# omrijsharon/FpyV

Measured on AMD Instinct MI355X. Metric: env-steps/sec at N=1.05M drones, dt=1ms; 1/2/4/8 GPU + CPU ref, higher is better.
Workload: dtype f32

## Files before the change

__graft_entry__.py:

```python
import os
import subprocess
import sys

REPO = os.path.dirname(os.path.abspath(__file__))
if REPO not in sys.path:
    sys.path.insert(0, REPO)

HIP_SRC = os.path.join(REPO, "fpyv_amd", "csrc", "fpv_hip.hip")
HIP_SRCS = [HIP_SRC, os.path.join(REPO, "fpyv_amd", "csrc", "fpv_phys.hip"), os.path.join(REPO, "fpyv_amd", "csrc", "fpv_gate.hip"),
            os.path.join(REPO, "fpyv_amd", "csrc", "fpv_range.hip")]
HIP_SRCS_ALL = HIP_SRCS + [os.path.join(REPO, "fpyv_amd", "csrc", "fpv_depth.hip")]
HIP_SRCS_BUILD = HIP_SRCS_ALL + [os.path.join(REPO, "fpyv_amd", "csrc", "fpv_chase.hip")]
HIP_SRCS_LINK = HIP_SRCS_BUILD + [os.path.join(REPO, "fpyv_amd", "csrc", "fpv_pursuit.hip")]
HIP_SRCS_PNS = HIP_SRCS_LINK + [os.path.join(REPO, "fpyv_amd", "csrc", "fpv_pns.hip")]
HIP_LIB = os.path.join(REPO, "fpyv_amd", "libfpv_hip.so")
HIPCC_FLAGS = ["-O3", "--offload-arch=gfx950", "-ffp-contract=off", "-fno-slp-vectorize", "-std=c++17", "-shared",
               "-fPIC", "-Wall", "-Wextra", "-mllvm", "-amdgpu-kernarg-preload-count=6"]


def _stale(target, sources):
    if not os.path.isfile(target):
        return True
    t = os.path.getmtime(target)
    return any(os.path.getmtime(s) > t for s in sources)


def build(force: bool = False) -> None:
    csrc = os.path.join(REPO, "fpyv_amd", "csrc")
    deps = [os.path.join(csrc, f) for f in os.listdir(csrc)] + [os.path.join(REPO, "include", "fpv_abi.h")]
    if force or _stale(HIP_LIB, deps):
        hipcc = os.environ.get("HIPCC", "/opt/rocm/bin/hipcc")
        subprocess.run([hipcc] + HIPCC_FLAGS + ["-o", HIP_LIB] + HIP_SRCS_PNS, check=True)
    subprocess.run(["make", "-C", os.path.join(REPO, "oracle")] + (["-B"] if force else []), check=True,
                   stdout=subprocess.DEVNULL)
    import fpyv_amd
    from fpyv_amd import _lib
    L = _lib.lib()
    missing = [s for s in _lib.EXPORTS if not hasattr(L, s)]
    assert not missing, f"libfpv_hip.so lacks {missing}"
    assert fpyv_amd.__version__


def smoke() -> None:
    import numpy as np
    import torch
    from fpyv_amd import load_params, sticks
    from fpyv_amd.env import DroneBatch
    from oracle import lane_model, oracle
    sys.path.insert(0, os.path.join(REPO, "tests"))
    from parity import assert_parity, soa_vs_oracle

    assert torch.cuda.is_available(), "smoke() needs a GPU"
    p = load_params(fps=1000)
    n, steps = 256, 200
    acts = sticks.ema_noise(steps, range(n), seed=7)
    a = torch.from_numpy(acts).to("cuda:0")
    env, fused = DroneBatch(p, n, device="cuda:0"), DroneBatch(p, n, device="cuda:0")
    env.reset(); fused.reset()
    for t in range(steps):
        env.step(a[t], return_imu=False)
    fused.rollout(a)
    torch.cuda.synchronize()
    got = env.state.cpu().numpy()
    assert torch.equal(env.state, fused.state), "k-step kernel != k single steps"

# ... 14 lines not shown
```

fpyv_amd/_lib.py:

```python
from __future__ import annotations

import ctypes as C
import os
from typing import Optional


_HERE = os.path.dirname(os.path.abspath(__file__))
LIB_PATH = os.path.join(_HERE, "libfpv_hip.so")

FPV_ABI_VERSION = 9
FPV_OK = 0
FPV_MODE_DRONE, FPV_MODE_RACER = 0, 1
FPV_DRONE_ROWS, FPV_RACER_ROWS = 14, 29
FPV_FLAG_AUTO_RESET = 1
FPV_FLAG_GROUND = 2
FPV_FLAG_FP16_STATE = 4
FPV_FLAG_STICK_NOISE = 8
FPV_FLAG_RESET_JITTER = 16
RESET_POSE_ROWS = 10
FPV_PHYS_ROWS = 13
FPV_PHYS_INPUTS = 10
PHYS_IN_MASS, PHYS_IN_C3, PHYS_IN_CD_X, PHYS_IN_RATES_LAG, PHYS_IN_THRUST_LAG = 0, 1, 5, 8, 9
FPV_MAX_GATES = 64
FPV_GATE_FLOATS = 16
GATE_SHAPES = {"rectangle": 0, "circle": 1, "half_circle": 2}
GATE_EVENT_NONE, GATE_EVENT_PASS, GATE_EVENT_MISS, GATE_EVENT_FINISH = 0, 1, 2, 3
GATE_OBS_ROWS = 6
FPV_MAX_RAYS = 32
FPV_DEPTH_MAX_SIDE = 128
DEPTH_ENCODINGS = {"metres": 0, "u8": 1}
FPV_CHASE_MAX_SIDE = 16384
CHASE_FRAMES = {"world": 0, "drone": 1}
CHASE_MODES = {"level": 0, "frontarget": 1}
FPV_TGT_ROWS = 8
TGT_CX, TGT_CY, TGT_CZ, TGT_PATH_R, TGT_RADIUS, TGT_PREV_DIST, TGT_COUNT, TGT_SPAWNS = range(8)
FPV_TGT_FRESH = 0x80000000
FPV_PURSUIT_OBS = 7
FPV_PURSUIT_MAX_RESOLUTION = 65536
FPV_HALF_PAIR_ROWS = 5
FPV_HALF_HALVES = 11
FPV_OBS_AOS_DIM = 16

PX, PY, PZ, VX, VY, VZ, QW, QX, QY, QZ, RX, RY, RZ, THRUST = range(14)
R_OMEGA, R_IERR, R_LERR, R_FIRST, R_OMEGA_LO, R_IERR_LO, R_DFILT = 10, 13, 16, 19, 20, 23, 26

EXPORTS = ("fpv_abi_version", "fpv_sizeof", "fpv_state_rows", "fpv_algorithmic_bytes", "fpv_handle_algorithmic_bytes", "fpv_create", "fpv_destroy",
           "fpv_reset", "fpv_step", "fpv_rollout", "fpv_step_n", "fpv_rollout_graph", "fpv_return_triple", "fpv_widen_state", "fpv_set_params", "fpv_set_step_counter", "fpv_get_step_counter", "fpv_set_rotation", "fpv_get_rotation", "fpv_recommended_ld",
           "fpv_recommended_ld_device", "fpv_check_cache_model", "fpv_device_cache_model", "fpv_get_cache_model",
           "fpv_diag_stream_copy", "fpv_diag_stream_copy_wide", "fpv_diag_busy", "fpv_diag_xcd_map", "fpv_pid_reset", "fpv_pid_call", "fpv_comm_unique_id", "fpv_comm_create", "fpv_comm_destroy", "fpv_comm_info",
           "fpv_allgather_done", "fpv_allgather_f32", "fpv_last_error",
           "fpv_error_name", "fpv_encoding_id", "fpv_reset_pose_sample",
           "fpv_physics_rows", "fpv_physics_derive", "fpv_physics_sample", "fpv_set_physics", "fpv_get_physics",
           "fpv_gates_derive", "fpv_set_gates", "fpv_gate_eval",
           "fpv_rays_derive", "fpv_range_scan", "fpv_range_eval",
           "fpv_camera_derive", "fpv_depth_render", "fpv_depth_eval",
           "fpv_chase_derive", "fpv_chase_guide", "fpv_chase_eval",
           "fpv_pursuit_derive", "fpv_pursuit_sample", "fpv_pursuit_step", "fpv_pursuit_reset", "fpv_pursuit_eval",
           "fpv_pns_derive", "fpv_pns_guide", "fpv_pns_eval")


class FpvParams(C.Structure):
    _fields_ = [
        ("struct_size", C.c_uint32), ("mode", C.c_uint32), ("flags", C.c_uint32), ("racer_omega_dt", C.c_uint32),
        ("dt", C.c_double), ("gravity", C.c_double), ("mass", C.c_double), ("max_rates", C.c_double),
        ("rates_transition_rate", C.c_double), ("thrust_transition_rate", C.c_double),
        ("thrust_poly", C.c_double * 4),
        ("drag_coefficients", C.c_double * 3), ("cross_section_areas", C.c_double * 3),
        ("air_density", C.c_double),
        ("motor_xy", (C.c_double * 2) * 4),
        ("init_position", C.c_double * 3), ("init_velocity", C.c_double * 3), ("init_quat", C.c_double * 4),
        ("ceiling", C.c_double), ("goal", C.c_double * 3),
        ("racer_mass", C.c_double), ("racer_inertia", C.c_double * 3), ("racer_pid", (C.c_double * 3) * 3),
        ("racer_velocity_damping", C.c_double),
        ("motor_radius", C.c_double), ("ground_spring", C.c_double), ("ground_damping", C.c_double),
        ("noise_transition", C.c_double), ("noise_gain", C.c_double),
        ("noise_seed", C.c_uint64), ("drone_id_offset", C.c_uint64),
        ("racer_pid_variant", C.c_uint32), ("_reserved0", C.c_uint32),
        ("pid_integral_clip", C.c_double), ("pid_min_output", C.c_double), ("pid_max_output", C.c_double),
        ("pid_derivative_transition_rate", C.c_double),
        ("reset_pos_range", (C.c_double * 3) * 2), ("reset_vel_range", (C.c_double * 3) * 2),
# ... 211 lines not shown

class FpvError(RuntimeError):
    def __init__(self, code: int, name: str, msg: str):
        super().__init__(f"{name} ({code}): {msg}")
        self.code, self.name = code, name


_lib: Optional[C.CDLL] = None


def lib() -> C.CDLL:
    global _lib
    if _lib is not None:
        return _lib
    if not os.path.isfile(LIB_PATH):
        raise ImportError(f"{LIB_PATH} is missing - build it with `python -c 'import __graft_entry__ as g; g.build()'` "
                          "(hipcc --offload-arch=gfx950).  fpyv_amd has no CPU fallback.")
    import torch
    L = C.CDLL(LIB_PATH, mode=C.RTLD_LOCAL)
    vp, i64, pp, pb = C.c_void_p, C.c_int64, C.POINTER(FpvParams), C.POINTER(FpvBuffers)
    L.fpv_abi_version.restype = C.c_int
    L.fpv_state_rows.argtypes = [C.c_int]
    L.fpv_algorithmic_bytes.argtypes = [C.c_int]
    L.fpv_handle_algorithmic_bytes.argtypes = [vp]
    L.fpv_create.argtypes = [pp, i64, C.c_int, C.POINTER(vp)]
    L.fpv_destroy.argtypes = [vp]
    L.fpv_destroy.restype = None
    L.fpv_reset.argtypes = [vp, pb, vp, vp, vp, vp, vp]
    L.fpv_step.argtypes = [vp, pb, vp]
    L.fpv_rollout.argtypes = [vp, pb, C.c_int, i64, i64, vp]
    L.fpv_rollout_graph.argtypes = [vp, pb, C.c_int, i64, i64, vp]
    L.fpv_step_n.argtypes = [vp, pb, C.c_int, i64, i64, vp]
    L.fpv_return_triple.argtypes = [vp, pb, vp, vp, vp, vp]
    L.fpv_widen_state.argtypes = [vp, pb, vp, i64, vp]
    L.fpv_set_params.argtypes = [vp, pp]
    L.fpv_set_step_counter.argtypes = [vp, C.c_uint64]
    L.fpv_get_step_counter.argtypes = [vp, C.POINTER(C.c_uint64)]
    L.fpv_set_rotation.argtypes = [vp, C.c_int64]
    L.fpv_get_rotation.argtypes = [vp, C.POINTER(C.c_int64)]
    L.fpv_recommended_ld.argtypes = [i64]
    L.fpv_recommended_ld.restype = i64
    L.fpv_recommended_ld_device.argtypes = [i64, C.c_int]
    L.fpv_recommended_ld_device.restype = i64
    L.fpv_check_cache_model.argtypes = [C.c_char_p, C.c_int, i64, C.POINTER(FpvCacheModel)]
    L.fpv_device_cache_model.argtypes = [C.c_int, C.POINTER(FpvCacheModel)]
    L.fpv_get_cache_model.argtypes = [vp, C.POINTER(FpvCacheModel)]
    L.fpv_diag_stream_copy.argtypes = [vp, vp, i64, vp]
    L.fpv_diag_stream_copy_wide.argtypes = [vp, vp, i64, vp]
    L.fpv_diag_busy.argtypes = [C.c_double, vp]
    L.fpv_diag_xcd_map.argtypes = [vp, i64, vp]
    L.fpv_comm_unique_id.argtypes = [vp]
    L.fpv_comm_create.argtypes = [vp, C.c_int, C.c_int, C.c_int, C.POINTER(vp)]
    L.fpv_comm_destroy.argtypes = [vp]
    L.fpv_comm_destroy.restype = None
    L.fpv_comm_info.argtypes = [vp, C.POINTER(C.c_int), C.POINTER(C.c_int), C.POINTER(C.c_int)]
    L.fpv_allgather_done.argtypes = [vp, vp, vp, i64, vp]
    L.fpv_allgather_f32.argtypes = [vp, vp, vp, i64, vp]
    L.fpv_pid_reset.argtypes = [vp, i64, i64, vp, C.c_int, vp]
    L.fpv_pid_call.argtypes = [C.POINTER(FpvPidParams), vp, i64, i64, vp, vp, C.c_float, vp, vp, C.c_int, vp]
    L.fpv_last_error.restype = C.c_char_p
    L.fpv_error_name.argtypes = [C.c_int]
    L.fpv_error_name.restype = C.c_char_p
    L.fpv_encoding_id.argtypes = [C.c_int]
    L.fpv_encoding_id.restype = C.c_char_p
    L.fpv_sizeof.argtypes = [C.c_int]
    L.fpv_reset_pose_sample.argtypes = [pp, C.c_uint64, C.c_uint64, C.c_int, vp, vp]
# ... 51 lines not shown
```

fpyv_amd/csrc/fpv_hip.hip:

```cpp
#include <hip/hip_runtime.h>

#include <dlfcn.h>
#include <math.h>
#include <stdint.h>
#include <stdio.h>
#include <stdlib.h>
#include <string.h>

#include <algorithm>
#include <mutex>
#include <new>
#include <string>
#include <vector>
#include <type_traits>

#include "../../include/fpv_abi.h"
#include "fpv_addr.h"
#include "fpv_exp.h"
#include "fpv_derive.h"
#include "fpv_math.h"
#include "fpv_kernels.h"
#include "fpv_range.h"
#include "fpv_depth.h"
#include "fpv_chase.h"
// ... 668 lines not shown
    fpv_params_t P;
    int64_t n;
    int device;
    int mode;
    FpvResetJitter rj;
    uint64_t launches;
    int64_t rot_blocks = 0, start_block = 0, rot_request = -1;
    fpv_cache_model_t cache;
    hipGraph_t graph = nullptr;
    hipGraphExec_t graph_exec = nullptr;
    std::vector<hipGraphNode_t> graph_nodes;
    std::string graph_shape_key, graph_ptr_key;
    const float* phys = nullptr;
    int64_t phys_ld = 0;
    int phys_rows_last = 0;
    bool gates = false;
    FpvGateArgs ga = {};
};

extern "C" __attribute__((weak, visibility("hidden"))) void* fpv_phys_step_kernel(int noise, int obj);
extern "C" __attribute__((weak, visibility("hidden"))) void* fpv_phys_roll_kernel(int noise, int obj);
extern "C" __attribute__((weak, visibility("hidden"))) void* fpv_gate_step_kernel(void);
extern "C" __attribute__((weak, visibility("hidden"))) void* fpv_gate_roll_kernel(int noise, int obj);
extern "C" __attribute__((weak, visibility("hidden"))) void* fpv_gate_reset_kernel_fn(void);
extern "C" __attribute__((weak, visibility("hidden"))) void* fpv_range_scan_kernel_fn(void);
extern "C" __attribute__((weak, visibility("hidden"))) void* fpv_depth_render_kernel_fn(int u8);
extern "C" __attribute__((weak, visibility("hidden"))) void* fpv_chase_kernel_fn(int pixel);
extern "C" __attribute__((weak, visibility("hidden"))) void fpv_chase_eval_host(const FpvChaseArgs* A, const float* p, const float* v, const float* q);
extern "C" __attribute__((weak, visibility("hidden"))) void* fpv_pns_kernel_fn(int pixel);
extern "C" __attribute__((weak, visibility("hidden"))) void fpv_pns_eval_host(const FpvPnsArgs* A, const float* p, const float* v, const float* q);
extern "C" __attribute__((weak, visibility("hidden"))) void* fpv_pursuit_kernel_fn(int guide, int reset);
extern "C" __attribute__((weak, visibility("hidden"))) void fpv_pursuit_eval_host(const FpvPursuitArgs* A, const float* p, const float* v, const float* q,
                                                                                  int guide, int reset);

namespace {

enum Family { kPlain, kFp16, kAos, kRacer, kTable, kGate };

int check_combination(const fpv_env* h, Family f, const fpv_buffers_t* b)
{
    struct Rule { bool hit; const char* with; };
    const bool table = f == kTable;
    const auto refuse = [&](std::initializer_list<Rule> rules) -> int {
        for (const Rule& r : rules)
            if (r.hit) return fail(FPV_EINVAL, std::string(table ? "a physics table" : "a gate course") + " cannot be combined with " + r.with);
        return FPV_OK;
    };
    if (!b)
        return refuse({{h->mode != FPV_MODE_DRONE, "Racer mode"}, {(h->K.flags & FPV_FLAG_FP16_STATE) != 0, "fp16 state (FPV_FLAG_FP16_STATE)"},
                       table ? Rule{h->gates, "a gate course (fpv_set_gates)"} : Rule{h->phys != nullptr, "a physics table (fpv_set_physics)"}});
    return refuse({{b->pos_comp != nullptr, "Kahan rows (pos_comp)"}, {b->rotation_override != nullptr, "the guidance override (rotation_override)"},
                   {b->obs_aos != nullptr, "the AoS head (obs_aos)"},
                   {!table && (h->K.flags & FPV_FLAG_STICK_NOISE) && b->objects && b->objects->count > 0, "stick noise AND an object list (either one alone is served)"}});
}

int check_object_count(const fpv_objects_t* in, bool most)
{
    if (in && (in->count < 0 || in->count > FPV_MAX_OBJECTS))
        return fail(FPV_EINVAL, "objects.count out of range" + (most ? " (at most " + std::to_string(FPV_MAX_OBJECTS) + " objects)" : std::string()));
    return FPV_OK;
}

int check_object_types(const fpv_objects_t* in)
{
    for (int k = 0; in && k < in->count; ++k)
        if (in->obj[k].type < FPV_OBJ_GROUND || in->obj[k].type > FPV_OBJ_SPHERE) return fail(FPV_EINVAL, "unknown object type");
// ... 155 lines not shown
};

typedef void (*StepKernel)(float*, const int64_t, const float4*, const int64_t, uint16_t*, const int64_t, const FpvK, const FpvBufD);
typedef void (*RollKernel)(const FpvRollArgs);
typedef void (*GateResetKernel)(uint32_t*, const uint8_t*, const uint8_t*, const uint32_t, const int64_t);
inline int64_t step_grid(int64_t n) { return (n + 8 * kStepBlock - 1) / (8 * kStepBlock) * 8; }

const StepKernel kDroneStep[2][2][2] = {
    {{fpv_drone_step_kernel<false, false, false>, fpv_drone_step_kernel<false, false, true>},
     {fpv_drone_step_kernel<false, true, false>, fpv_drone_step_kernel<false, true, true>}},
    {{fpv_drone_step_kernel<true, false, false>, fpv_drone_step_kernel<true, false, true>},
     {fpv_drone_step_kernel<true, true, false>, fpv_drone_step_kernel<true, true, true>}}};
const StepKernel kDroneStepOverride[2] = {fpv_drone_step_kernel<false, false, false, true>, fpv_drone_step_kernel<false, true, false, true>};
const RollKernel kDroneRoll[2][2][2] = {
    {{fpv_drone_rollout_kernel<false, false, false>, fpv_drone_rollout_kernel<false, false, true>},
     {fpv_drone_rollout_kernel<false, true, false>, fpv_drone_rollout_kernel<false, true, true>}},
    {{fpv_drone_rollout_kernel<true, false, false>, fpv_drone_rollout_kernel<true, false, true>},
     {fpv_drone_rollout_kernel<true, true, false>, fpv_drone_rollout_kernel<true, true, true>}}};
const RollKernel kDroneRollSq[2][2] = {
    {fpv_drone_rollout_kernel<false, false, false, true>, fpv_drone_rollout_kernel<false, false, true, true>},
    {fpv_drone_rollout_kernel<true, false, false, true>, fpv_drone_rollout_kernel<true, false, true, true>}};
const StepKernel kRacerStep[2][2] = {{fpv_racer_step_kernel<false, false>, fpv_racer_step_kernel<false, true>},
                                     {fpv_racer_step_kernel<true, false>, fpv_racer_step_kernel<true, true>}};
const RollKernel kRacerRoll[2][2] = {{fpv_racer_rollout_kernel<false, false>, fpv_racer_rollout_kernel<false, true>},
                                     {fpv_racer_rollout_kernel<true, false>, fpv_racer_rollout_kernel<true, true>}};

enum GraphRoute { kReplay, kToStepN, kToRollout };
struct Plan {
    Family family;
    void* step;
    void* roll;
    bool ground = false;
    GraphRoute graph = kReplay;
};

template <class... P> void* entry(void (*kernel)(P...)) { return reinterpret_cast<void*>(kernel); }

Plan plan_launch(const fpv_env* h, const FpvBufD& d)
{
    const bool noise = (h->K.flags & FPV_FLAG_STICK_NOISE) != 0, fp16 = (h->K.flags & FPV_FLAG_FP16_STATE) != 0;
    const bool obj = d.objs.count > 0, kahan = d.pos_comp != nullptr, aos = d.obs_aos != nullptr, ground = (h->K.flags & FPV_FLAG_GROUND) != 0;
    const bool wide = h->K.r_wide != 0, pidv = h->K.r_pid_variant != 0;
    const bool reset = h->mode == FPV_MODE_DRONE && (d.reset_pose != nullptr || (h->K.flags & FPV_FLAG_RESET_JITTER) != 0);
    const bool sq = !obj && h->K.motor_square && !ground && !reset;
    Plan p;
    if (h->gates) p = {kGate, noise || obj ? nullptr : fpv_gate_step_kernel(), fpv_gate_roll_kernel(noise, obj)};
    else if (h->phys) p = {kTable, fpv_phys_step_kernel(noise, obj), fpv_phys_roll_kernel(noise, obj), ground || obj};
    else if (h->mode != FPV_MODE_DRONE) p = {kRacer, entry(kRacerStep[wide][pidv]), entry(kRacerRoll[wide][pidv])};
    else if (fp16) p = {kFp16, entry(fpv_drone_step_h_kernel), entry(fpv_drone_rollout_h_kernel)};
    else p = {aos ? kAos : kPlain, entry(aos ? fpv_drone_step_aos_kernel : d.rot_over ? kDroneStepOverride[obj] : kDroneStep[noise][obj][kahan]),
              entry(sq ? kDroneRollSq[noise][kahan] : kDroneRoll[noise][obj][kahan])};
    if (reset && !aos) p.step = nullptr;
    p.graph = noise || fp16 || !p.step ? kToStepN : reset ? kToRollout : kReplay;
    return p;
}

void launched(fpv_env* h, const Plan& p, int k)
{
    h->launches += (uint64_t)k;
    if (p.family == kTable) h->phys_rows_last = p.ground ? FPV_PHYS_ROWS : FPV_PHYS_ROWS - 2;
}

int launch_roll(fpv_env* h, const Plan& p, const FpvBufD& d, const FpvRoll& R, hipStream_t s, const char* what)
{
    FpvRollArgs a = {h->K, d, h->n, R};
    a.B.step = h->launches;
    FpvRollPhysArgs pa;
    FpvRollGateArgs ga;
    void* arg = &a;
    if (p.family == kTable) { pa = {a, h->phys, p.ground ? 1 : 0, 0}; arg = &pa; }
    if (p.family == kGate) { ga = {a, h->ga}; arg = &ga; }
    const int rc = launch_args(what, p.roll, blocks_for(h->n, kStepBlock), dim3(kStepBlock), s, &arg);
    if (rc == FPV_OK) launched(h, p, R.k);
    return rc;
}

struct StepLaunch {
    FpvBufD d;
    FpvK K;
    int64_t n_start;
    void* slot5;
    FpvGateArgs ga;
    void* args[9];
    hipKernelNodeParams np;
    StepLaunch(const fpv_env* h, const Plan& p, const FpvBufD& dt, int64_t start)
        : d(dt), K(h->K), n_start(h->n | (start << 32) | (p.ground ? kPhysGroundBit : 0)),
          slot5(p.family == kGate ? (void*)h->ga.word : p.family == kTable ? (void*)const_cast<float*>(h->phys) : (void*)dt.state_h),
          ga(h->ga), args{&d.state, &d.ld, &d.action, &d.action_ld, &slot5, &n_start, &K, &d, &ga}
    {
        memset(&np, 0, sizeof(np));
        np.func = p.step; np.kernelParams = args;
        np.gridDim = dim3((unsigned)step_grid(h->n)); np.blockDim = dim3(kStepBlock);
    }
    StepLaunch(const StepLaunch&) = delete;
    StepLaunch& operator=(const StepLaunch&) = delete;
};

int64_t rotation_blocks(const fpv_env* h, const FpvBufD* d);

int launch_step(fpv_env* h, const Plan& p, const FpvBufD& d, hipStream_t s)
{
    if (!p.step) return launch_roll(h, p, d, FpvRoll{1, 0, 0, 0, 0}, s, "step kernel launch");
    const int64_t nblk = step_grid(h->n);
    h->rot_blocks = rotation_blocks(h, &d);
    const int64_t start = h->rot_blocks > 0 ? h->start_block % nblk : 0;
    StepLaunch L(h, p, d, start);
    L.d.step = h->launches;
    const int rc = launch_args("step kernel launch", L.np.func, L.np.gridDim, L.np.blockDim, s, L.np.kernelParams);
    if (rc != FPV_OK) return rc;
    launched(h, p, 1);
    if (h->rot_blocks > 0) h->start_block = (start + nblk - h->rot_blocks % nblk) % nblk;
    return FPV_OK;
}

template <class... T> std::string bytes_of(const T&... v)
{
    std::string s;
    (s.append(reinterpret_cast<const char*>(&v), sizeof(v)), ...);
    return s;
}

constexpr int kModelXcds = 8, kModelComputeUnits = 256;
constexpr int64_t kModelL2BytesPerXcd = (int64_t)4 << 20;
constexpr int64_t kInfinityCacheBytes = (int64_t)256 << 20;
constexpr int64_t kL2Bytes = (int64_t)kModelXcds * kModelL2BytesPerXcd;

void check_cache_model(const char* arch, int compute_units, int64_t l2_bytes, fpv_cache_model_t* m)
{
    memset(m, 0, sizeof(*m));
    m->struct_size = (uint32_t)sizeof(*m);
    m->compute_units = compute_units;
    m->l2_bytes_per_xcd = l2_bytes;
    snprintf(m->arch, sizeof(m->arch), "%s", arch ? arch : "");
    std::string why;
    if (strncmp(m->arch, "gfx950", 6) != 0 || (m->arch[6] != '\0' && m->arch[6] != ':'))
        why = std::string("architecture '") + m->arch + "' is not gfx950";
    else if (compute_units != kModelComputeUnits)
        why = "the process sees " + std::to_string(compute_units) + " compute units, not " + std::to_string(kModelComputeUnits)
              + " (a compute partition of the chip? the model is eight XCDs of 32 CUs in single-partition mode)";
// ... 983 lines not shown
            const double o = l2_set_overflow(4 * c, blocks);
            if (o < kL2OverflowOk) return c;
            if (o < best) { best = o; best_ld = c; }
        }
    return best_ld;
}

int fpv_reset(fpv_handle_t h, const fpv_buffers_t* b, const uint8_t* mask, const float* position,
              const float* velocity, const float* ypr_deg, void* stream)
{
    int rc = check_buffers(h, b, false);
    if (rc != FPV_OK) return rc;
    const DeviceGuard dev(h->device);
    if (dev.rc != FPV_OK) return dev.rc;
    FpvBufD d = to_device_view(h, b);
    d.step = h->launches;
    rc = launch("reset kernel launch", fpv_reset_kernel, blocks_for(h->n, kBlock), dim3(kBlock), (hipStream_t)stream, h->K, d,
                h->mode, mask, position, velocity, ypr_deg, h->n);
    if (rc != FPV_OK || !h->gates) return rc;
    return launch("gate word reset launch", reinterpret_cast<GateResetKernel>(fpv_gate_reset_kernel_fn()), blocks_for(h->n, kBlock), dim3(kBlock),
                  (hipStream_t)stream, h->ga.word, mask, h->ga.start, h->ga.K.count, h->n);
}

int fpv_step(fpv_handle_t h, const fpv_buffers_t* b, void* stream)
{
    int rc = check_buffers(h, b, true);
    if (rc != FPV_OK) return rc;
    const DeviceGuard dev(h->device);
    if (dev.rc != FPV_OK) return dev.rc;
    const FpvBufD d = to_device_view(h, b);
    return launch_step(h, plan_launch(h, d), d, (hipStream_t)stream);
}

namespace {

void drop_graph(fpv_env* h)
{
    if (h->graph_exec) { (void)hipGraphExecDestroy(h->graph_exec); h->graph_exec = nullptr; }
    if (h->graph) { (void)hipGraphDestroy(h->graph); h->graph = nullptr; }
    h->graph_nodes.clear();
    h->graph_shape_key.clear();
    h->graph_ptr_key.clear();
}

FpvBufD graph_step_view(const fpv_buffers_t* b, const FpvBufD& d0, int t, int64_t action_stride, int64_t out_stride)
{
    FpvBufD d = d0;
    if (b->action) d.action = reinterpret_cast<const float4*>(b->action + (int64_t)t * action_stride);
    if (out_stride) {
        if (b->reward) d.reward = b->reward + (int64_t)t * out_stride;
        if (b->done) d.done = b->done + (int64_t)t * out_stride;
    }
    if (b->done_bits) d.done_bits = reinterpret_cast<unsigned long long*>(b->done_bits) + (int64_t)t * b->done_bits_stride;
    return d;
}

}

int fpv_rollout(fpv_handle_t h, const fpv_buffers_t* b, int k, int64_t action_stride, int64_t out_stride,
                void* stream)
{
    int rc = check_buffers(h, b, true);
    if (rc != FPV_OK) return rc;
    if (k < 0) return fail(FPV_EINVAL, "k must be >= 0");
    if (action_stride % 4) return fail(FPV_EALIGN, "action_stride must keep 16-byte alignment");
    if (b->rotation_override) return fail(FPV_EINVAL, "the guidance override is a per-step input: use fpv_step");
// ... 329 lines not shown
```

fpyv_amd/csrc/fpv_kernels.h:

```cpp
#pragma once

#include <hip/hip_runtime.h>

#include <stdint.h>

#include <type_traits>

#include "../../include/fpv_abi.h"
#include "fpv_addr.h"
#include "fpv_exp.h"
#include "fpv_math.h"
#include "fpv_gate.h"

namespace {

constexpr int kBlock = 256;
constexpr int kStepBlock = FPV_EXP_BLOCK;
static_assert(kStepBlock % 64 == 0 && kStepBlock >= 64 && kStepBlock <= 1024, "whole wave64s");

struct FpvBufD {
    float* state;
    int64_t ld;
    const float4* action;
    float* reward;
// ... 224 lines not shown
    return p;
}

__device__ __forceinline__ void apply_reset_source_k(uint32_t i, uint64_t t, FpvDroneState& s)
{
    float pose[10] = {s.px, s.py, s.pz, s.vx, s.vy, s.vz, s.q.w, s.q.x, s.q.y, s.q.z};
    FpvArgsPtr A = fpv_args_after(s.px);
    const float* tab = A->B.reset_pose;
    if (tab) {
        const int64_t ld = A->B.ld;
#pragma unroll
        for (int r = 0; r < 10; ++r) pose[r] = row_at(ROW(tab, r, ld), i);
    }
    if (A->K.flags & FPV_FLAG_RESET_JITTER) {
#pragma unroll
        for (uint32_t b = 0; b < 3; ++b) {
            const FpvArgsPtr V = fpv_args_after(pose[3 * b]);
            const float lo[3] = {V->B.rj.lo[3 * b], V->B.rj.lo[3 * b + 1], V->B.rj.lo[3 * b + 2]};
            const float span[3] = {V->B.rj.span[3 * b], V->B.rj.span[3 * b + 1], V->B.rj.span[3 * b + 2]};
            fpv_reset_jitter_block(lo, span, V->B.rj.seed_lo, V->B.rj.seed_hi, (((uint64_t)V->K.noise.id_hi << 32) | V->K.noise.id_lo) + i,
                                   V->B.step + t, 0u, b, pose);
        }
    }
    s.px = pose[0]; s.py = pose[1]; s.pz = pose[2]; s.vx = pose[3]; s.vy = pose[4]; s.vz = pose[5];
    s.q.w = pose[6]; s.q.x = pose[7]; s.q.y = pose[8]; s.q.z = pose[9];
}

struct FpvRollPhysArgs { FpvRollArgs A; const float* phys; int32_t ground; int32_t pad; };
constexpr int64_t kPhysGroundBit = (int64_t)1 << 31;

struct FpvGateArgs { const fpv_gate_v4* tab; uint32_t* word; float* obs; int64_t obs_ld; const uint8_t* start; FpvGateK K; };
struct FpvRollGateArgs { FpvRollArgs A; FpvGateArgs G; };

}
```

fpyv_amd/env.py:

```python
from __future__ import annotations

import ctypes as C
from typing import Any, Dict, Optional, Sequence, Tuple

import numpy as np
import torch

from . import _lib
from .params import DroneParams, MODE_DRONE, MODE_RACER, load_params


STATE_H_ENCODING = "abi5: v f16+5-bit low words, q smallest-three 15-bit fixed point, rates/thrust f16"
NOISE_GENERATOR = "abi5: philox4x32-7, table-driven inverse normal CDF"
_FIRST_ABI_WITH_ENCODING_LABEL = 6
CHECKPOINT_LAYOUT = "columns"


def _round_up(x: int, m: int) -> int:
    return (x + m - 1) // m * m


def _set_wind(buf: _lib.FpvBuffers, wind: Sequence[float]) -> None:
    w = buf.wind
    w[0], w[1], w[2] = float(wind[0]), float(wind[1]), float(wind[2])
# ... 29 lines not shown
    @property
    def _auto_reset(self) -> bool:
        return bool(self._cparams.flags & _lib.FPV_FLAG_AUTO_RESET)

    def set_params(self, params: DroneParams, auto_reset: Optional[bool] = None) -> None:
        cp = self._pack(params, self._auto_reset if auto_reset is None else auto_reset)
        _lib.check(self._L.fpv_set_params(self._handle, C.byref(cp)))
        self.params, self._cparams = params, cp

    def set_step_counter(self, step: int) -> None:
        if not 0 <= int(step) < 2 ** 64:
            raise ValueError("the step counter is an unsigned 64-bit integer")
        _lib.check(self._L.fpv_set_step_counter(self._handle, int(step)))
        self._steps_launched = int(step)

    def close(self) -> None:
        if getattr(self, "_handle", None) is not None and self._handle.value:
            self._L.fpv_destroy(self._handle)
            self._handle = C.c_void_p()

    def __del__(self):
        try:
            self.close()
        except Exception:
            pass

    def _stream(self) -> int:
        try:
            return torch._C._cuda_getCurrentRawStream(self._dev_index)
        except AttributeError:
            return torch.cuda.current_stream(self.device).cuda_stream

    def _step_raw(self, action: Any, wind: Optional[Sequence[float]] = None,
                  stream: Optional[torch.cuda.Stream] = None) -> None:
        b = self._buf
        self._keepalive, b.action, b.action_ld = self._sticks(action, stream)
        if wind is not None:
            _set_wind(b, wind)
        rc = self._fpv_step(self._handle, self._buf_ref, self._stream() if stream is None else stream.cuda_stream)
        if rc < 0:
            _lib.check(rc)
        self._steps_launched = (self._steps_launched + 1) & 0xFFFFFFFFFFFFFFFF

    def _sticks(self, action: Any, stream: Optional[torch.cuda.Stream] = None,
                block: bool = False) -> Tuple[Optional[torch.Tensor], Optional[int], int]:
        if action is None:
            if not self.stick_noise:
                raise ValueError("action=None is only meaningful with stick_noise=True (pure noise sticks)")
            return None, None, 0
        if action is self._last_action and action.data_ptr() == self._last_action_ptr and action.shape == self._ashape:
            return action, self._last_action_ptr, 0
        self._last_action = None
        if type(action) is torch.Tensor and action.dtype is torch.float32 and action.device == self._dev:
            if action.shape == self._ashape and action.is_contiguous():
                self._last_action, self._last_action_ptr = action, action.data_ptr()
                return action, self._last_action_ptr, 0
            if (not block and action.dim() == 2 and action.shape[0] == 4 and action.shape[1] == self.n != 4
                    and action.stride(1) == 1 and action.stride(0) >= self.n):
                return action, action.data_ptr(), action.stride(0)
        elif (torch.is_tensor(action) and action.dtype in (torch.float16, torch.bfloat16, torch.float64)
              and action.device == self._dev
              and (block or (action.shape == self._ashape if self._coerce else type(action) is torch.Tensor))):
            return self._sticks(self._cast_sticks(action, stream), stream, block)
        if block:
            if torch.is_tensor(action) and action.dtype is torch.float32 and action.is_contiguous() and action.device == self._dev:
                return action, action.data_ptr(), 0
            raise ValueError("actions must be a contiguous float32 tensor on the env's device (float16 / bfloat16 / float64 "
                             "tensors there are cast once per call)")
        if not self._coerce:
            raise ValueError(f"a partition's action is a float32 tensor on the env's device, [{self.n}, 4] contiguous rows or "
                             f"[4, {self.n}] with unit column stride (slices of a full-size tensor qualify)")
        action = self._coerce_action(action)
# ... 702 lines not shown
                    fn = self._L.fpv_rollout
                else:
                    fn = self._L.fpv_step_n
            else:
                fn = self._L.fpv_rollout
            _lib.check(fn(self._handle, C.byref(b), int(k), stride, out_stride, self._stream()))
            self._steps_launched = (self._steps_launched + int(k)) & 0xFFFFFFFFFFFFFFFF
            self._keepalive = actions
        finally:
            b.reward, b.done = saved

    @property
    def position(self) -> torch.Tensor:
        return self.rows_f32(_lib.PX, _lib.PZ + 1)

    @property
    def velocity(self) -> torch.Tensor:
        return self.rows_f32(_lib.VX, _lib.VZ + 1)

    @property
    def quaternion(self) -> torch.Tensor:
        return self.rows_f32(_lib.QW, _lib.QZ + 1)

    @property
    def rotation_matrix(self) -> torch.Tensor:
        if self.mode == MODE_DRONE and not self.fp16_state:
            return self._return_triple(False)[0].transpose(-1, -2)
        return quat_to_matrix(self.quaternion)

    def _return_triple(self, with_accel: bool):
        f32 = dict(dtype=torch.float32, device=self.device)
        rt, gyro = torch.empty((self.n, 3, 3), **f32), torch.empty((self.n, 3, 3), **f32)
        acc = torch.empty((self.n, 3), **f32) if with_accel else None
        _lib.check(self._L.fpv_return_triple(self._handle, self._buf_ref, rt.data_ptr(), gyro.data_ptr(),
                                             acc.data_ptr() if acc is not None else None, self._stream()))
        return rt, gyro, acc


class _Partition(_Handle):

    _coerce = False

    def __init__(self, parent: "_Batch", lo: int, hi: int, stream: Optional[torch.cuda.Stream]):
        if lo % 128 or not lo < hi <= parent.n:
            raise ValueError("a partition starts at a multiple of 128 drones and is not empty")
        self.parent, self.lo, self.hi = parent, lo, hi
        self.stream = stream if stream is not None else torch.cuda.Stream(device=parent.device)
        super().__init__(parent.params, hi - lo, parent.device, parent._dev_index, parent._auto_reset,
                         dict(parent._pack_kw, drone_id_offset=int(parent._pack_kw["drone_id_offset"]) + lo))
        self.rebind()

    def rebind(self) -> None:
        pb, b, lo = self.parent._buf, self._buf, self.lo
        off = lambda base, elem_bytes, per_drone=1: (base + lo * elem_bytes * per_drone) if base else None
        b.state, b.ld = off(pb.state, 4), pb.ld
        b.reward, b.done = off(pb.reward, 4), off(pb.done, 1)
        b.done_bits = (pb.done_bits + (lo // 64) * 8) if pb.done_bits else None
        b.accel, b.pos_comp, b.noise_state = off(pb.accel, 4), off(pb.pos_comp, 4), off(pb.noise_state, 4)
        b.reset_pose = off(pb.reset_pose, 4)
        b.ep_return, b.ep_length = off(pb.ep_return, 4), off(pb.ep_length, 4)
        b.last_return, b.last_length = off(pb.last_return, 4), off(pb.last_length, 4)
        b.action_out, b.obs_aos = off(pb.action_out, 4, 4), off(pb.obs_aos, 4, _lib.FPV_OBS_AOS_DIM)
        b.wind[0], b.wind[1], b.wind[2] = pb.wind[0], pb.wind[1], pb.wind[2]
        b.rounding_seed, b.objects = pb.rounding_seed, pb.objects
        if pb.state_h:
            b.state_h = pb.state_h + 4 * lo
# ... 99 lines not shown


class DroneBatch(_Batch):

    def __init__(self, params: Any = None, num_envs: int = 1, device: Any = "cuda:0", **kw):
        params = as_drone_params(params, mode=MODE_DRONE)
        kw.setdefault("with_accel", True)
        super().__init__(params, num_envs, device, **kw)
        self.dt = params.dt
        self.max_rates = params.max_rates
        self.mass, self.gravity = params.mass, params.gravity
        self.throttle2thrust = params.thrust_from_stick
        self.thrust2throttle = params.stick_from_thrust
        self.min_throttle_in_force = params.min_throttle_in_force
        self.max_throttle_in_force = params.max_throttle_in_force
        self._force_multiplier_pid = None

    @property
    def force_multiplier_pid(self):
        if self._force_multiplier_pid is None:
            from .pid import PID
            kw = dict(self.params.force_multiplier_pid)
            kw["min_output"], kw["max_output"] = self.min_throttle_in_force, self.max_throttle_in_force
            self._force_multiplier_pid = PID(**kw, dt=self.dt, num_envs=self.n, device=self.device)
        return self._force_multiplier_pid

    def reset(self, position=None, velocity=None, ypr=None, mask=None) -> None:
        self._reset_raw(mask=mask, position=position, velocity=velocity, ypr=ypr)
        if self._force_multiplier_pid is not None:
            self._force_multiplier_pid.reset(mask)
        self._pns_reset(mask)

    def step(self, action, wind_velocity_vector=None, object_list=(), rotation_matrix=None, thrust_force=None,
             return_imu: bool = True):
        if action is None and not self.stick_noise:
            raise ValueError("action=None reads a physical joystick in the reference; pass stick values")
        if rotation_matrix is None and self._objects is None and not object_list:
            self._step_raw(action, wind_velocity_vector)
        else:
            try:
                self._set_override(rotation_matrix, thrust_force)
                self._set_objects(object_list)
                self._step_raw(action, wind_velocity_vector)
            finally:
                self._buf.rotation_override = self._buf.thrust_override = None
                self._override_keep = None
        if self._pursuit is not None:
            self._pursuit_step_raw()
        if not return_imu:
            return None
        if not self.fp16_state:
            return self._return_triple(self.accel is not None)
        R = self.rotation_matrix
        rates = self.rows_f32(_lib.RX, _lib.RZ + 1)
        gyro = euler_zyx_matrix(rates)
        acc = self.accel[:, :self.n].t() if self.accel is not None else None
        return R.transpose(-1, -2), gyro, acc

    @property
    def euler_angles(self) -> torch.Tensor:
        return matrix_to_euler_zyx(self.rotation_matrix)

    def get_gravity_force_in_drone_ref_frame(self) -> torch.Tensor:
        g = torch.tensor([0.0, 0.0, -9.81 * self.mass], dtype=torch.float32, device=self.device)
        return self.rotation_matrix @ g

    def _set_override(self, rotation_matrix, thrust_force) -> None:
        if rotation_matrix is None:
            return
        if thrust_force is None:
            raise TypeError("rotation_matrix= needs thrust_force= (kinematics.thrust_vector(None, R) raises in the reference)")
        f32 = dict(dtype=torch.float32, device=self.device)
        R = torch.as_tensor(np.asarray(rotation_matrix, dtype=np.float32) if not torch.is_tensor(rotation_matrix)
                            else rotation_matrix, **f32)
        if R.shape == (3, 3):
            R = R.expand(self.n, 3, 3)
        if R.shape != (self.n, 3, 3):
            raise ValueError(f"rotation_matrix must be [3, 3] or [{self.n}, 3, 3], got {tuple(R.shape)}")
        f = torch.as_tensor(np.asarray(thrust_force, dtype=np.float32) if not torch.is_tensor(thrust_force)
                            else thrust_force, **f32).reshape(-1)
        if f.numel() == 1:
            f = f.expand(self.n)
        if f.shape != (self.n,):
            raise ValueError(f"thrust_force must be a scalar or [{self.n}], got {tuple(f.shape)}")
        self._override_keep = (R.reshape(self.n, 9).contiguous(), f.contiguous())
# ... 347 lines not shown
```

include/fpv_abi.h:

```cpp
#ifndef FPV_ABI_H
#define FPV_ABI_H

#include <stdint.h>

#ifdef __cplusplus
extern "C" {
#endif

#define FPV_ABI_VERSION 9

enum {
    FPV_OK = 0,
    FPV_EINVAL = -1,
    FPV_EHIP = -2,
    FPV_ENODEV = -3,
    FPV_EALIGN = -4,
    FPV_EPARAM = -5
};

enum { FPV_MODE_DRONE = 0, FPV_MODE_RACER = 1 };

enum {
    FPV_PX = 0, FPV_PY, FPV_PZ,
    FPV_VX, FPV_VY, FPV_VZ,
// ... 122 lines not shown
    FPV_PHYS_IN_RATES_LAG, FPV_PHYS_IN_THRUST_LAG,
    FPV_PHYS_INPUTS
};
int fpv_physics_rows(void);
int fpv_physics_derive(const fpv_params_t* base, int64_t n, const double* inputs ,
                       float* out_rows , int64_t out_ld);
int fpv_physics_sample(const fpv_params_t* base, uint64_t seed, uint64_t global_id0, int64_t n,
                       const double* ranges , double* out_inputs);

typedef struct fpv_env* fpv_handle_t;

int fpv_abi_version(void);
int fpv_sizeof(int which);
int fpv_state_rows(int mode);
int fpv_algorithmic_bytes(int mode);
int fpv_handle_algorithmic_bytes(fpv_handle_t h);

int fpv_create(const fpv_params_t* params, int64_t n, int device, fpv_handle_t* out);
void fpv_destroy(fpv_handle_t h);

int fpv_reset(fpv_handle_t h, const fpv_buffers_t* b, const uint8_t* mask, const float* position,
              const float* velocity, const float* ypr_deg, void* stream);

int fpv_step(fpv_handle_t h, const fpv_buffers_t* b, void* stream);

int fpv_rollout(fpv_handle_t h, const fpv_buffers_t* b, int k, int64_t action_stride,
                int64_t out_stride, void* stream);

int fpv_step_n(fpv_handle_t h, const fpv_buffers_t* b, int k, int64_t action_stride,
               int64_t out_stride, void* stream);

int fpv_return_triple(fpv_handle_t h, const fpv_buffers_t* b, float* rt, float* gyro, float* acc, void* stream);

int fpv_widen_state(fpv_handle_t h, const fpv_buffers_t* b, float* out, int64_t out_ld, void* stream);

int fpv_set_step_counter(fpv_handle_t h, uint64_t step);
int fpv_get_step_counter(fpv_handle_t h, uint64_t* step);

int fpv_set_rotation(fpv_handle_t h, int64_t drones);
int fpv_get_rotation(fpv_handle_t h, int64_t* drones);

typedef struct fpv_cache_model_t {
    uint32_t struct_size;
    int32_t matches;
    int32_t compute_units;
    int32_t xcds;
    int64_t l2_bytes_per_xcd;
    int64_t infinity_cache_bytes;
    char arch[64];
    char reason[256];
} fpv_cache_model_t;
int fpv_check_cache_model(const char* arch, int compute_units, int64_t l2_bytes_per_xcd, fpv_cache_model_t* out);
int fpv_device_cache_model(int device, fpv_cache_model_t* out);
int fpv_get_cache_model(fpv_handle_t h, fpv_cache_model_t* out);

int fpv_rollout_graph(fpv_handle_t h, const fpv_buffers_t* b, int k, int64_t action_stride,
                      int64_t out_stride, void* stream);

int fpv_set_params(fpv_handle_t h, const fpv_params_t* params);

int fpv_set_physics(fpv_handle_t h, const float* table, int64_t ld);
int fpv_get_physics(fpv_handle_t h, const float** table, int64_t* ld);

#define FPV_MAX_GATES 64
#define FPV_GATE_FLOATS 16
enum { FPV_GATE_RECTANGLE = 0, FPV_GATE_CIRCLE = 1, FPV_GATE_HALF_CIRCLE = 2 };
// ... 221 lines not shown
```

Before: 53.72 billion.

## Fuse IMU return-triple computation into the drone step kernel

Adds an fpv_step_imu entry point and a fused step kernel that computes R^T, gyro matrix and acceleration right after the physics step. Outputs are staged through LDS per wave and written with coalesced nontemporal vector stores. This avoids a separate return-triple kernel launch and its re-read of the state from memory when step() returns IMU data. It applies only on the plain fp32 drone path with aligned outputs and no done/return buffers, and it adds LDS use and a __syncthreads per block, which may lower occupancy.

```diff
diff --git a/__graft_entry__.py b/__graft_entry__.py
--- a/__graft_entry__.py
+++ b/__graft_entry__.py
@@ -13,6 +13,7 @@
 HIP_SRCS_BUILD = HIP_SRCS_ALL + [os.path.join(REPO, "fpyv_amd", "csrc", "fpv_chase.hip")]
 HIP_SRCS_LINK = HIP_SRCS_BUILD + [os.path.join(REPO, "fpyv_amd", "csrc", "fpv_pursuit.hip")]
 HIP_SRCS_PNS = HIP_SRCS_LINK + [os.path.join(REPO, "fpyv_amd", "csrc", "fpv_pns.hip")]
+HIP_SRCS_IMU = HIP_SRCS_PNS + [os.path.join(REPO, "fpyv_amd", "csrc", "fpv_imu.hip")]
 HIP_LIB = os.path.join(REPO, "fpyv_amd", "libfpv_hip.so")
 HIPCC_FLAGS = ["-O3", "--offload-arch=gfx950", "-ffp-contract=off", "-fno-slp-vectorize", "-std=c++17", "-shared",
                "-fPIC", "-Wall", "-Wextra", "-mllvm", "-amdgpu-kernarg-preload-count=6"]
@@ -30,7 +31,7 @@
     deps = [os.path.join(csrc, f) for f in os.listdir(csrc)] + [os.path.join(REPO, "include", "fpv_abi.h")]
     if force or _stale(HIP_LIB, deps):
         hipcc = os.environ.get("HIPCC", "/opt/rocm/bin/hipcc")
-        subprocess.run([hipcc] + HIPCC_FLAGS + ["-o", HIP_LIB] + HIP_SRCS_PNS, check=True)
+        subprocess.run([hipcc] + HIPCC_FLAGS + ["-o", HIP_LIB] + HIP_SRCS_IMU, check=True)
     subprocess.run(["make", "-C", os.path.join(REPO, "oracle")] + (["-B"] if force else []), check=True,
                    stdout=subprocess.DEVNULL)
     import fpyv_amd
diff --git a/fpyv_amd/_lib.py b/fpyv_amd/_lib.py
--- a/fpyv_amd/_lib.py
+++ b/fpyv_amd/_lib.py
@@ -45,7 +45,7 @@
 R_OMEGA, R_IERR, R_LERR, R_FIRST, R_OMEGA_LO, R_IERR_LO, R_DFILT = 10, 13, 16, 19, 20, 23, 26
 
 EXPORTS = ("fpv_abi_version", "fpv_sizeof", "fpv_state_rows", "fpv_algorithmic_bytes", "fpv_handle_algorithmic_bytes", "fpv_create", "fpv_destroy",
-           "fpv_reset", "fpv_step", "fpv_rollout", "fpv_step_n", "fpv_rollout_graph", "fpv_return_triple", "fpv_widen_state", "fpv_set_params", "fpv_set_step_counter", "fpv_get_step_counter", "fpv_set_rotation", "fpv_get_rotation", "fpv_recommended_ld",
+           "fpv_reset", "fpv_step", "fpv_rollout", "fpv_step_n", "fpv_rollout_graph", "fpv_return_triple", "fpv_step_imu", "fpv_widen_state", "fpv_set_params", "fpv_set_step_counter", "fpv_get_step_counter", "fpv_set_rotation", "fpv_get_rotation", "fpv_recommended_ld",
            "fpv_recommended_ld_device", "fpv_check_cache_model", "fpv_device_cache_model", "fpv_get_cache_model",
            "fpv_diag_stream_copy", "fpv_diag_stream_copy_wide", "fpv_diag_busy", "fpv_diag_xcd_map", "fpv_pid_reset", "fpv_pid_call", "fpv_comm_unique_id", "fpv_comm_create", "fpv_comm_destroy", "fpv_comm_info",
            "fpv_allgather_done", "fpv_allgather_f32", "fpv_last_error",
@@ -323,6 +323,7 @@
     L.fpv_rollout_graph.argtypes = [vp, pb, C.c_int, i64, i64, vp]
     L.fpv_step_n.argtypes = [vp, pb, C.c_int, i64, i64, vp]
     L.fpv_return_triple.argtypes = [vp, pb, vp, vp, vp, vp]
+    L.fpv_step_imu.argtypes = [vp, pb, vp, vp, vp, vp]
     L.fpv_widen_state.argtypes = [vp, pb, vp, i64, vp]
     L.fpv_set_params.argtypes = [vp, pp]
     L.fpv_set_step_counter.argtypes = [vp, C.c_uint64]
diff --git a/fpyv_amd/csrc/fpv_hip.hip b/fpyv_amd/csrc/fpv_hip.hip
--- a/fpyv_amd/csrc/fpv_hip.hip
+++ b/fpyv_amd/csrc/fpv_hip.hip
@@ -724,6 +724,7 @@
 extern "C" __attribute__((weak, visibility("hidden"))) void* fpv_pursuit_kernel_fn(int guide, int reset);
 extern "C" __attribute__((weak, visibility("hidden"))) void fpv_pursuit_eval_host(const FpvPursuitArgs* A, const float* p, const float* v, const float* q,
                                                                                   int guide, int reset);
+extern "C" __attribute__((weak, visibility("hidden"))) void* fpv_imu_step_kernel_fn(int acc);
 
 namespace {
 
@@ -945,11 +946,12 @@
     void* roll;
     bool ground = false;
     GraphRoute graph = kReplay;
+    bool imu = false;
 };
 
 template <class... P> void* entry(void (*kernel)(P...)) { return reinterpret_cast<void*>(kernel); }
 
-Plan plan_launch(const fpv_env* h, const FpvBufD& d)
+Plan plan_launch(const fpv_env* h, const FpvBufD& d, const FpvImuArgs* imu = nullptr)
 {
     const bool noise = (h->K.flags & FPV_FLAG_STICK_NOISE) != 0, fp16 = (h->K.flags & FPV_FLAG_FP16_STATE) != 0;
     const bool obj = d.objs.count > 0, kahan = d.pos_comp != nullptr, aos = d.obs_aos != nullptr, ground = (h->K.flags & FPV_FLAG_GROUND) != 0;
@@ -965,6 +967,12 @@
               entry(sq ? kDroneRollSq[noise][kahan] : kDroneRoll[noise][obj][kahan])};
     if (reset && !aos) p.step = nullptr;
     p.graph = noise || fp16 || !p.step ? kToStepN : reset ? kToRollout : kReplay;
+    const auto aligned16 = [](const void* q) { return (reinterpret_cast<uintptr_t>(q) & 15u) == 0; };
+    if (imu && fpv_imu_step_kernel_fn && p.family == kPlain && p.step == entry(kDroneStep[0][0][0]) && !d.ep_return && !d.done_bits
+        && aligned16(imu->rt) && aligned16(imu->gyro) && aligned16(imu->acc)) {
+        p.step = fpv_imu_step_kernel_fn(imu->acc != nullptr);
+        p.imu = true;
+    }
     return p;
 }
 
@@ -994,12 +1002,14 @@
     int64_t n_start;
     void* slot5;
     FpvGateArgs ga;
+    FpvImuArgs imu;
     void* args[9];
     hipKernelNodeParams np;
-    StepLaunch(const fpv_env* h, const Plan& p, const FpvBufD& dt, int64_t start)
+    StepLaunch(const fpv_env* h, const Plan& p, const FpvBufD& dt, int64_t start, const FpvImuArgs* out = nullptr)
         : d(dt), K(h->K), n_start(h->n | (start << 32) | (p.ground ? kPhysGroundBit : 0)),
           slot5(p.family == kGate ? (void*)h->ga.word : p.family == kTable ? (void*)const_cast<float*>(h->phys) : (void*)dt.state_h),
-          ga(h->ga), args{&d.state, &d.ld, &d.action, &d.action_ld, &slot5, &n_start, &K, &d, &ga}
+          ga(h->ga), imu(out ? *out : FpvImuArgs{nullptr, nullptr, nullptr}),
+          args{&d.state, &d.ld, &d.action, &d.action_ld, &slot5, &n_start, &K, &d, p.imu ? (void*)&imu : (void*)&ga}
     {
         memset(&np, 0, sizeof(np));
         np.func = p.step; np.kernelParams = args;
@@ -1011,13 +1021,13 @@
 
 int64_t rotation_blocks(const fpv_env* h, const FpvBufD* d);
 
-int launch_step(fpv_env* h, const Plan& p, const FpvBufD& d, hipStream_t s)
+int launch_step(fpv_env* h, const Plan& p, const FpvBufD& d, hipStream_t s, const FpvImuArgs* imu = nullptr)
 {
     if (!p.step) return launch_roll(h, p, d, FpvRoll{1, 0, 0, 0, 0}, s, "step kernel launch");
     const int64_t nblk = step_grid(h->n);
     h->rot_blocks = rotation_blocks(h, &d);
     const int64_t start = h->rot_blocks > 0 ? h->start_block % nblk : 0;
-    StepLaunch L(h, p, d, start);
+    StepLaunch L(h, p, d, start, imu);
     L.d.step = h->launches;
     const int rc = launch_args("step kernel launch", L.np.func, L.np.gridDim, L.np.blockDim, s, L.np.kernelParams);
     if (rc != FPV_OK) return rc;
@@ -2067,6 +2077,25 @@
     return launch_step(h, plan_launch(h, d), d, (hipStream_t)stream);
 }
 
+int fpv_step_imu(fpv_handle_t h, const fpv_buffers_t* b, float* rt, float* gyro, float* acc, void* stream)
+{
+    int rc = check_buffers(h, b, true);
+    if (rc != FPV_OK) return rc;
+    if (!rt || !gyro) return fail(FPV_EINVAL, "null argument");
+    if (h->mode != FPV_MODE_DRONE || (h->K.flags & FPV_FLAG_FP16_STATE))
+        return fail(FPV_EINVAL, "fpv_step_imu returns the fp32 drone state's triple (Drone.step's return value)");
+    if (acc && !b->accel) return fail(FPV_EINVAL, "R @ acceleration needs fpv_buffers_t.accel (the step kernel writes it there)");
+    const DeviceGuard dev(h->device);
+    if (dev.rc != FPV_OK) return dev.rc;
+    const FpvBufD d = to_device_view(h, b);
+    const FpvImuArgs out = {rt, gyro, acc};
+    const Plan p = plan_launch(h, d, &out);
+    rc = launch_step(h, p, d, (hipStream_t)stream, &out);
+    if (rc != FPV_OK || p.imu) return rc;
+    return launch("return-triple kernel launch", fpv_return_triple_kernel, blocks_for(h->n, kBlock), dim3(kBlock), (hipStream_t)stream,
+                  b->state, b->ld, b->accel, rt, gyro, acc, h->n);
+}
+
 namespace {
 
 void drop_graph(fpv_env* h)
diff --git a/fpyv_amd/csrc/fpv_imu.hip b/fpyv_amd/csrc/fpv_imu.hip
--- /dev/null
+++ b/fpyv_amd/csrc/fpv_imu.hip
@@ -0,0 +1,99 @@
+#include <hip/hip_runtime.h>
+
+#include <stdint.h>
+
+#include <type_traits>
+
+#include "../../include/fpv_abi.h"
+#include "fpv_addr.h"
+#include "fpv_exp.h"
+#include "fpv_math.h"
+#include "fpv_kernels.h"
+
+namespace {
+
+struct FpvStepImuArgs { FpvStepArgs S; FpvImuArgs I; };
+__device__ __forceinline__ const FpvStepImuArgs& fpv_step_imu_args_again()
+{
+    typedef const __attribute__((address_space(4))) FpvStepImuArgs* P4;
+    P4 p = (P4)__builtin_amdgcn_kernarg_segment_ptr();
+    asm volatile("" : "+s"(p));
+    return *(const FpvStepImuArgs*)p;
+}
+
+template <int PER>
+__device__ __forceinline__ void st_wave_tile(const float* tile, float* out, int lane, int count)
+{
+    constexpr int kF4 = 16 * PER;
+#pragma unroll
+    for (int j = 0; j * 64 < kF4; ++j) {
+        const int f4 = j * 64 + lane, at = f4 * 4;
+        if (f4 >= kF4 || at >= count) continue;
+        const float* src = tile + at;
+        if (at + 4 <= count) {
+            fpv_v4f v4;
+            v4.x = src[0]; v4.y = src[1]; v4.z = src[2]; v4.w = src[3];
+            __builtin_nontemporal_store(v4, reinterpret_cast<fpv_v4f*>(out) + f4);
+        } else {
+            for (int c = 0; at + c < count; ++c) __builtin_nontemporal_store(src[c], out + at + c);
+        }
+    }
+}
+
+template <bool ACC>
+__global__ __launch_bounds__(kStepBlock) void fpv_drone_step_imu_kernel(FPV_STEP_PARAMS, const FpvImuArgs I_)
+{
+    (void)K; (void)I_;
+    FPV_STEP_VIEW;
+    constexpr int kWaves = kStepBlock / 64;
+    __shared__ __attribute__((aligned(16))) float t_rt[kWaves][64 * 9];
+    __shared__ __attribute__((aligned(16))) float t_gyro[kWaves][64 * 9];
+    __shared__ __attribute__((aligned(16))) float t_acc[ACC ? kWaves : 1][64 * 3];
+    FPV_STEP_INDEX;
+    const bool live = i < n;
+    const int lane = threadIdx.x & 63, wave = threadIdx.x >> 6;
+    FpvStepOut o;
+    o.done = false; o.reward = 0.0f; o.ax = o.ay = o.az = 0.0f;
+    if (live) {
+        FpvDroneState s;
+        const float4 a = ld_action_any(B.action, B.action_ld, i);
+        const FpvStepArgs* T = &fpv_step_args_again();
+        const FpvK Kt = T->K;
+        const float wind[3] = {T->B.wx, T->B.wy, T->B.wz};
+        __builtin_amdgcn_sched_barrier(0);
+        ld_drone(B.state, B.ld, i, s);
+        __builtin_amdgcn_sched_barrier(0);
+        o = fpv_drone_step_lane<false>(Kt, s, a.x, a.y, a.z, a.w, wind[0], wind[1], wind[2], &B_.objs, nullptr, nullptr, 0.0f);
+        if (B.accel) {
+            ST_OUT(row_at(ROW(B.accel, 0, B.ld), i), o.ax); ST_OUT(row_at(ROW(B.accel, 1, B.ld), i), o.ay); ST_OUT(row_at(ROW(B.accel, 2, B.ld), i), o.az);
+        }
+        if ((Kt.flags & FPV_FLAG_AUTO_RESET) && o.done) fpv_drone_reset_lane(Kt, s);
+        st_drone(B.state, B.ld, i, s);
+        float rt[9], gyro[9];
+        fpv_return_matrices(s.q, s.rx, s.ry, s.rz, rt, gyro);
+#pragma unroll
+        for (int k = 0; k < 9; ++k) { t_rt[wave][lane * 9 + k] = rt[k]; t_gyro[wave][lane * 9 + k] = gyro[k]; }
+        if (ACC) { t_acc[wave][lane * 3 + 0] = o.ax; t_acc[wave][lane * 3 + 1] = o.ay; t_acc[wave][lane * 3 + 2] = o.az; }
+    }
+    FpvBufD Bo = B;
+    Bo.done_bits = nullptr; Bo.ep_return = nullptr;
+    emit_outputs(Bo, i, live, o.reward, o.done);
+    __syncthreads();
+    const uint32_t wave_first = i - (uint32_t)lane;
+    if (wave_first >= n) return;
+    const int mine = (int)(n - wave_first < 64 ? n - wave_first : 64);
+    const FpvImuArgs& I = fpv_step_imu_args_again().I;
+    st_wave_tile<9>(t_rt[wave], I.rt + (int64_t)wave_first * 9, lane, mine * 9);
+    st_wave_tile<9>(t_gyro[wave], I.gyro + (int64_t)wave_first * 9, lane, mine * 9);
+    if (ACC) st_wave_tile<3>(t_acc[wave], I.acc + (int64_t)wave_first * 3, lane, mine * 3);
+}
+
+typedef void (*ImuStepFn)(float*, const int64_t, const float4*, const int64_t, uint16_t*, const int64_t, const FpvK, const FpvBufD, const FpvImuArgs);
+const ImuStepFn kImuStep[2] = {fpv_drone_step_imu_kernel<false>, fpv_drone_step_imu_kernel<true>};
+
+}
+
+extern "C" __attribute__((visibility("hidden"))) void* fpv_imu_step_kernel_fn(int acc)
+{
+    return reinterpret_cast<void*>(kImuStep[acc != 0]);
+}
diff --git a/fpyv_amd/csrc/fpv_kernels.h b/fpyv_amd/csrc/fpv_kernels.h
--- a/fpyv_amd/csrc/fpv_kernels.h
+++ b/fpyv_amd/csrc/fpv_kernels.h
@@ -280,4 +280,6 @@
 struct FpvGateArgs { const fpv_gate_v4* tab; uint32_t* word; float* obs; int64_t obs_ld; const uint8_t* start; FpvGateK K; };
 struct FpvRollGateArgs { FpvRollArgs A; FpvGateArgs G; };
 
-}
+struct FpvImuArgs { float* rt; float* gyro; float* acc; };
+
+}
diff --git a/fpyv_amd/env.py b/fpyv_amd/env.py
--- a/fpyv_amd/env.py
+++ b/fpyv_amd/env.py
@@ -85,12 +85,17 @@
             return torch.cuda.current_stream(self.device).cuda_stream
 
     def _step_raw(self, action: Any, wind: Optional[Sequence[float]] = None,
-                  stream: Optional[torch.cuda.Stream] = None) -> None:
+                  stream: Optional[torch.cuda.Stream] = None, imu: Optional[Tuple[Any, Any, Any]] = None) -> None:
         b = self._buf
         self._keepalive, b.action, b.action_ld = self._sticks(action, stream)
         if wind is not None:
             _set_wind(b, wind)
-        rc = self._fpv_step(self._handle, self._buf_ref, self._stream() if stream is None else stream.cuda_stream)
+        s = self._stream() if stream is None else stream.cuda_stream
+        if imu is None:
+            rc = self._fpv_step(self._handle, self._buf_ref, s)
+        else:
+            rc = self._L.fpv_step_imu(self._handle, self._buf_ref, imu[0].data_ptr(), imu[1].data_ptr(),
+                                      imu[2].data_ptr() if imu[2] is not None else None, s)
         if rc < 0:
             _lib.check(rc)
         self._steps_launched = (self._steps_launched + 1) & 0xFFFFFFFFFFFFFFFF
@@ -859,6 +864,25 @@
         f32 = dict(dtype=torch.float32, device=self.device)
         rt, gyro = torch.empty((self.n, 3, 3), **f32), torch.empty((self.n, 3, 3), **f32)
         acc = torch.empty((self.n, 3), **f32) if with_accel else None
+        return self._return_triple_into(rt, gyro, acc)
+
+    def _triple_out(self, out):
+        f32 = dict(dtype=torch.float32, device=self.device)
+        if out is None:
+            return (torch.empty((self.n, 3, 3), **f32), torch.empty((self.n, 3, 3), **f32),
+                    torch.empty((self.n, 3), **f32) if self.accel is not None else None)
+        rt, gyro, acc = out
+        for t, shape in ((rt, (self.n, 3, 3)), (gyro, (self.n, 3, 3)), (acc, (self.n, 3))):
+            if t is None and shape == (self.n, 3):
+                continue
+            if (not torch.is_tensor(t) or t.dtype != torch.float32 or tuple(t.shape) != shape or not t.is_contiguous()
+                    or t.device != self.state.device):
+                raise ValueError("out must be contiguous float32 tensors [n, 3, 3], [n, 3, 3], [n, 3] on the env's device")
+        if acc is not None and self.accel is None:
+            raise ValueError("out's acc needs the accel rows (with_accel=True)")
+        return rt, gyro, acc
+
+    def _return_triple_into(self, rt, gyro, acc):
         _lib.check(self._L.fpv_return_triple(self._handle, self._buf_ref, rt.data_ptr(), gyro.data_ptr(),
                                              acc.data_ptr() if acc is not None else None, self._stream()))
         return rt, gyro, acc
@@ -1024,16 +1048,20 @@
         self._pns_reset(mask)
 
     def step(self, action, wind_velocity_vector=None, object_list=(), rotation_matrix=None, thrust_force=None,
-             return_imu: bool = True):
+             return_imu: bool = True, out=None):
         if action is None and not self.stick_noise:
             raise ValueError("action=None reads a physical joystick in the reference; pass stick values")
+        imu = None
+        if return_imu and not self.fp16_state:
+            imu = self._triple_out(out)
+        fused = imu if self._pursuit is None else None
         if rotation_matrix is None and self._objects is None and not object_list:
-            self._step_raw(action, wind_velocity_vector)
+            self._step_raw(action, wind_velocity_vector, imu=fused)
         else:
             try:
                 self._set_override(rotation_matrix, thrust_force)
                 self._set_objects(object_list)
-                self._step_raw(action, wind_velocity_vector)
+                self._step_raw(action, wind_velocity_vector, imu=fused)
             finally:
                 self._buf.rotation_override = self._buf.thrust_override = None
                 self._override_keep = None
@@ -1041,8 +1069,8 @@
             self._pursuit_step_raw()
         if not return_imu:
             return None
-        if not self.fp16_state:
-            return self._return_triple(self.accel is not None)
+        if imu is not None:
+            return imu if fused is not None else self._return_triple_into(*imu)
         R = self.rotation_matrix
         rates = self.rows_f32(_lib.RX, _lib.RZ + 1)
         gyro = euler_zyx_matrix(rates)
diff --git a/include/fpv_abi.h b/include/fpv_abi.h
--- a/include/fpv_abi.h
+++ b/include/fpv_abi.h
@@ -178,6 +178,8 @@
 
 int fpv_return_triple(fpv_handle_t h, const fpv_buffers_t* b, float* rt, float* gyro, float* acc, void* stream);
 
+int fpv_step_imu(fpv_handle_t h, const fpv_buffers_t* b, float* rt, float* gyro, float* acc, void* stream);
+
 int fpv_widen_state(fpv_handle_t h, const fpv_buffers_t* b, float* out, int64_t out_ld, void* stream);
 
 int fpv_set_step_counter(fpv_handle_t h, uint64_t step);
```

After: 53.09 billion. 1.2% lower.
